# NyanCAD/CedarSim.jl

Hardware: AMD Instinct MI355X
Metric: newton_iters_per_sec (higher is better)
Workload: dtype f64

## Files before the change

### cedarsim.jl_amd/csrc/ch_persist.hpp

```cpp
#pragma once
#include <hip/hip_runtime.h>

#include "ch_kernels.hpp"

#ifdef CH_STAMPS
#define P_STAMP(slot) do { const unsigned long long now_ = __builtin_readcyclecounter(); pacc_[slot] += now_ - plast_; plast_ = now_; } while (0)
#else
#define P_STAMP(slot) do { } while (0)
#endif

namespace chip {

constexpr int PW = 4;
constexpr int P_MAXSRC = 64;
constexpr int P_NREC = 8;
constexpr int P_SCR = 64;
enum { PX_RUNNING = 0, PX_DONE = 1, PX_ROWS_FULL = 2, PX_ABORT = 3 };

struct TranCtl {
  double t, h;
  double tslot[8];
  int k, nhist, steps_at_order, reset_rate;
  int ibp, isave, status, exit_reason;
  long long nsaved, step;
// ... 29 lines not shown

struct PConst {
  const int* ci; const double* cd;
  __device__ int n_need() const { return ci[0]; }
  __device__ int n_ent() const { return ci[1]; }
  __device__ int n_pwl() const { return ci[2]; }
  __device__ const int* src_rec(int i) const { return ci + 4 + 3 * i; }
  __device__ const int* ent_ptr() const { return ci + 4 + 3 * n_need(); }
  __device__ const int* ent_idx() const { return ent_ptr() + n_ent() + 1; }
  __device__ const double* par(int i) const { return cd + 8 * i; }
  __device__ const double* ent_coef() const { return cd + 8 * n_need(); }
  __device__ const double* pwl_t() const { return ent_coef() + ent_ptr()[n_ent()]; }
  __device__ const double* pwl_y() const { return pwl_t() + n_pwl(); }
};

__device__ inline double p_pwl(const double* ts, const double* ys, int n, double t) {
  if (n == 0) return 0.0;
  int lo = 0, hi = n;
  while (lo < hi) { const int mid = (lo + hi) >> 1; if (ts[mid] < t) lo = mid + 1; else hi = mid; }
  int i = lo + 1;
  if (i <= n && ts[i - 1] == t) ++i;
  if (i <= 1) return ys[0];
  if (i > n) return ys[n - 1];
  const double y0 = ys[i - 2], y1 = ys[i - 1], t0 = ts[i - 2], t1 = ts[i - 1];
  if (y0 == y1) return y1;
  if (t1 == t0) return 0.5 * (y0 + y1);
  return y0 + (t - t0) * ((y1 - y0) / (t1 - t0));
}
__device__ inline double p_pwl4(double c0, double c1, double c2, double c3, double v1, double v2, double t) {
  int lb = (c0 < t) + (c1 < t) + (c2 < t) + (c3 < t);
  int i = lb + 1;
  const double tlb = lb == 0 ? c0 : lb == 1 ? c1 : lb == 2 ? c2 : c3;
  if (i <= 4 && tlb == t) ++i;
  if (i <= 1) return v1;
  if (i > 4) return v1;
  const double t0 = i == 2 ? c0 : i == 3 ? c1 : c2, t1 = i == 2 ? c1 : i == 3 ? c2 : c3;
  const double y0 = i == 2 ? v1 : v2, y1 = i == 4 ? v1 : v2;
  if (y0 == y1) return y1;
  if (t1 == t0) return 0.5 * (y0 + y1);
  return y0 + (t - t0) * ((y1 - y0) / (t1 - t0));
}
__device__ inline double p_source(const PConst& C, int i, double t) {
  const int* r = C.src_rec(i);
  const double* par = C.par(i);
  switch (r[0]) {
    case CH_SRC_DC: return par[0];
    case CH_SRC_PWL: return p_pwl(C.pwl_t() + r[1], C.pwl_y() + r[1], r[2], t);
    case CH_SRC_PULSE: {
      const double td = par[2], tr = par[3], tf = par[4], pw = par[5], per = par[6];
      const double tt = (per == per && fabs(per) < __builtin_inf()) ? fmod(t, per) : t;
      return p_pwl4(td, td + tr, td + tr + pw, td + tr + pw + tf, par[0], par[1], tt);
    }
    case CH_SRC_SIN: {
      const double vo = par[0], va = par[1], f = par[2], td = par[3], th = par[4], ph = par[5], nc = par[6];
      const double rad = 3.14159265358979323846 / 180.0;
      if (td < t && t < nc / f) return vo + va * exp(-(t - td) * th) * sin(fmod(360.0 * f * (t - td) + ph, 360.0) * rad);
      return vo + va * sin(fmod(ph, 360.0) * rad);
    }
  }
  return 0.0;
}

__device__ inline void p_source_piece(const PConst& C, int i, double t, double& t_lo, double& t_hi, double& y_lo, double& slope) {
  const int* r = C.src_rec(i);
  const double inf = __builtin_inf();
  t_lo = inf; t_hi = -inf; y_lo = 0.0; slope = 0.0;
  if (r[0] == CH_SRC_DC) { t_lo = -inf; t_hi = inf; y_lo = C.par(i)[0]; return; }
  if (r[0] != CH_SRC_PWL) return;
  const double* ts = C.pwl_t() + r[1]; const double* ys = C.pwl_y() + r[1];
  const int n = r[2];
  if (n == 0) { t_lo = -inf; t_hi = inf; return; }
  int lo = 0, hi = n;
  while (lo < hi) { const int mid = (lo + hi) >> 1; if (ts[mid] < t) lo = mid + 1; else hi = mid; }
  int k = lo + 1;
  if (k <= n && ts[k - 1] == t) ++k;
  if (k <= 1) { t_lo = -inf; t_hi = ts[0]; y_lo = ys[0]; return; }
  if (k > n) { t_lo = ts[n - 1]; t_hi = inf; y_lo = ys[n - 1]; return; }
  const double y0 = ys[k - 2], y1 = ys[k - 1], t0 = ts[k - 2], t1 = ts[k - 1];
  if (t1 == t0) return;
  t_lo = t0; t_hi = t1;
  if (y0 == y1) { y_lo = y1; slope = 0.0; } else { y_lo = y0; slope = (y1 - y0) / (t1 - t0); }
}

__device__ __forceinline__ void lds_fence() { asm volatile("s_waitcnt lgkmcnt(0)" ::: "memory"); }

__device__ __forceinline__ double ld_agent(const double* p) { return __hip_atomic_load(p, __ATOMIC_RELAXED, __HIP_MEMORY_SCOPE_AGENT); }
__device__ __forceinline__ void st_agent(double* p, double v) { __hip_atomic_store(p, v, __ATOMIC_RELAXED, __HIP_MEMORY_SCOPE_AGENT); }
__device__ __forceinline__ unsigned ld_agent_u(const unsigned* p) { return __hip_atomic_load(p, __ATOMIC_RELAXED, __HIP_MEMORY_SCOPE_AGENT); }

__device__ inline bool p_wait(const unsigned* cnt, unsigned target, unsigned* abort_flag, long long spin_ticks) {
  const long long t0 = wall_clock64();
  for (;;) {
    if (ld_agent_u(cnt) >= target) return true;
    if (ld_agent_u(abort_flag) != 0u) return false;
    if (wall_clock64() - t0 > spin_ticks) { __hip_atomic_store(abort_flag, 1u, __ATOMIC_RELAXED, __HIP_MEMORY_SCOPE_AGENT); return false; }
    __builtin_amdgcn_s_sleep(2);
  }
}

__device__ __forceinline__ double p_tree(double v, bool is_max) {
#pragma unroll
  for (int o = 8; o < 64; o <<= 1) { const double u = __shfl_xor(v, o); v = is_max ? fmax(v, u) : v + u; }
  return v;
}

typedef unsigned long long p_u64;
__device__ __forceinline__ p_u64 ld_gran(const p_u64* p) { return __hip_atomic_load(p, __ATOMIC_RELAXED, __HIP_MEMORY_SCOPE_AGENT); }
__device__ __forceinline__ void st_gran(p_u64* p, p_u64 v) { __hip_atomic_store(p, v, __ATOMIC_RELAXED, __HIP_MEMORY_SCOPE_AGENT); }
__device__ __forceinline__ double p_join(p_u64 gran, int lane) {
  const unsigned mine = (unsigned)gran, other = (unsigned)dpp_i<DPP_QP_1032>((int)mine);
  const unsigned lo = (lane & 1) ? other : mine, hi = (lane & 1) ? mine : other;
  return __hiloint2double((int)hi, (int)lo);
}
__device__ __forceinline__ p_u64 p_split(double v, int lane, unsigned gen) {
  const unsigned half = (lane & 1) ? (unsigned)__double2hiint(v) : (unsigned)__double2loint(v);
  return ((p_u64)gen << 32) | half;
}
__device__ __forceinline__ double p_rows4(double v, bool is_max, double* scr, int lane) {
  scr[lane] = v;
  asm volatile("s_waitcnt lgkmcnt(0)" ::: "memory");
  const int c = lane & 15;
  const double a0 = scr[c], a1 = scr[16 + c], a2 = scr[32 + c], a3 = scr[48 + c];
  asm volatile("s_waitcnt lgkmcnt(0)" ::: "memory");
  return is_max ? fmax(fmax(a0, a1), fmax(a2, a3)) : (a0 + a1) + (a2 + a3);
}
template <bool ALL_SUM = false>
__device__ inline bool p_grid_reduce(const PersistArgs& p, unsigned gen, const double* rec , double* part, double* summ,
                                     int* s_abort, int wave, int lane, int wg) {
  const int g16 = lane & 15, f = g16 >> 1, m4 = lane >> 4;
  const bool fmaxop = !ALL_SUM && ((f == 4) || (p.red_max && f < 3));
  if (lane < P_NREC) {
    double v = rec[0];
#pragma unroll
    for (int q = 1; q < P_NREC; ++q) v = (lane == q) ? rec[q] : v;
    part[wave * P_NREC + lane] = v;
  }
  __syncthreads();
  const int n_grp = p.n_wg < 8 ? p.n_wg : 8;
  const int grp = wg & 7;
  unsigned* abort_flag = p.counters + 9 * 32;
  p_u64* wrec = (p_u64*)p.wg_rec + (size_t)(gen & 1) * p.n_wg * 16;
  p_u64* grec = (p_u64*)p.grp_rec + (size_t)(gen & 1) * 8 * 16;
  double* scr = part + PW * P_NREC + P_NREC + 4;
  if (wave == 0) {
    bool ok = true;
    double v = part[f];
#pragma unroll
    for (int w = 1; w < PW; ++w) { const double u = part[w * P_NREC + f]; v = fmaxop ? fmax(v, u) : v + u; }
    if (p.n_wg > 1) {
      if (lane < 16) st_gran(wrec + (size_t)wg * 16 + g16, p_split(v, lane, gen));
      const long long t0 = wall_clock64();
      if (wg < n_grp) {
        const int members = (p.n_wg - grp + 7) >> 3;
        p_u64 x[8];
        for (;;) {
          bool all = true;
          const unsigned ab = ld_agent_u(abort_flag);
#pragma unroll
          for (int q = 0; q < 8; ++q) {
            const int mm = q * 4 + m4;
            x[q] = mm < members ? ld_gran(wrec + (size_t)(grp + 8 * mm) * 16 + g16) : ((p_u64)gen << 32);
            all = all && (unsigned)(x[q] >> 32) == gen;
          }
          if (__all(all)) break;
          if (ab != 0u) { ok = false; break; }
          if (wall_clock64() - t0 > p.spin_ticks) { __hip_atomic_store(abort_flag, 1u | (gen << 8), __ATOMIC_RELAXED, __HIP_MEMORY_SCOPE_AGENT); ok = false; break; }
          __builtin_amdgcn_s_sleep(1);
        }
        double acc = (m4 < members) ? p_join(x[0], lane) : 0.0;
#pragma unroll
        for (int q = 1; q < 8; ++q) {
          const double u = (q * 4 + m4 < members) ? p_join(x[q], lane) : 0.0;
          acc = fmaxop ? fmax(acc, u) : acc + u;
        }
        acc = p_rows4(acc, fmaxop, scr, lane);
        if (lane < 16) st_gran(grec + (size_t)grp * 16 + g16, p_split(acc, lane, gen));
      }
      p_u64 y[2];
      for (;;) {
        bool all = true;
        const unsigned ab = ok ? ld_agent_u(abort_flag) : 1u;
#pragma unroll
        for (int q = 0; q < 2; ++q) {
          const int gg = q * 4 + m4;
          y[q] = (ok && gg < n_grp) ? ld_gran(grec + (size_t)gg * 16 + g16) : ((p_u64)gen << 32);
          all = all && (unsigned)(y[q] >> 32) == gen;
        }
        if (__all(all) || !ok) break;
        if (ab != 0u) { ok = false; break; }
        if (wall_clock64() - t0 > p.spin_ticks) { __hip_atomic_store(abort_flag, 2u | (gen << 8), __ATOMIC_RELAXED, __HIP_MEMORY_SCOPE_AGENT); ok = false; break; }
        __builtin_amdgcn_s_sleep(1);
      }
      double acc = (m4 < n_grp) ? p_join(y[0], lane) : 0.0;
      { const double u = (4 + m4 < n_grp) ? p_join(y[1], lane) : 0.0; acc = fmaxop ? fmax(acc, u) : acc + u; }
      v = p_rows4(acc, fmaxop, scr, lane);
    }
    if (lane < 16 && !(lane & 1)) summ[f] = v;
    if (lane == 0) *s_abort = ok ? 0 : 1;
  }
  __syncthreads();
  return *s_abort == 0;
}

__device__ __forceinline__ double p_coef(double tau0, const double* tsl, int head, int kk, int np, int nkm1, int nkp1, bool lte, double hh, int lane, double& a0) {
  double tau[9];
  tau[0] = tau0;
#pragma unroll
  for (int i = 1; i < 9; ++i) tau[i] = tsl[(head - (i - 1)) & 7];
  const int set = lane >> 3, j = lane & 7;
  const double tj = j == 0 ? tau0 : tsl[(head - (j - 1)) & 7];
  const int n = set == 0 ? kk : set == 1 ? np : set == 2 ? nkm1 : set == 3 ? nkp1 : 0;
  const int lo = set == 0 ? 0 : 1;
  double num = 1.0, den = 1.0;
#pragma unroll
  for (int i = 0; i < 8; ++i) {
    const bool in_n = i >= 1 && i <= n && i != j, in_d = i >= lo && i <= n && i != j;
    num *= in_n ? tau[0] - tau[i] : 1.0;
    den *= in_d ? tj - tau[i] : 1.0;
  }
  if (!(set <= 3 && j >= 1 && j <= n)) { num = 0.0; den = 1.0; }
  double tk0 = tau[1], tk1 = tau[1], tk2 = tau[1];
#pragma unroll
  for (int i = 1; i < 9; ++i) { tk0 = (kk == i) ? tau[i] : tk0; tk1 = (kk + 1 == i) ? tau[i] : tk1; tk2 = (kk + 2 == i) ? tau[i] : tk2; }
  if (set == 4) {
    if (j >= 1 && j <= 5) { num = j <= kk ? 1.0 : 0.0; den = tau[0] - tj; }
    else if (j == 6) { num = lte ? hh : 0.0; den = tau[0] - tk1; }
    else if (j == 7) { num = nkm1 > 0 ? hh : 0.0; den = tau[0] - tk0; }
  } else if (set == 5 && j == 0) { num = nkp1 > 0 ? hh : 0.0; den = tau[0] - tk2; }
  if (num == 0.0) den = 1.0;
  const double q = num / den;
  a0 = bcast(row_sum<16>((set == 4 && j >= 1 && j <= 5) ? q : 0.0), 32);
  return q;
}

enum { PM_LOCKSTEP = 0, PM_OWN = 1, PM_BORDER = 2 };
template <int NC, bool PAIR, int MODE = PM_LOCKSTEP, bool WIDE = false>
__global__ __launch_bounds__(PW * 64, 1) void tran_persistent_kernel(const PersistArgs p) {
  typedef StampLayout<WIDE> SL;
  extern __shared__ double lds[];
  __shared__ int s_abort;
  __shared__ double s_bdec[4];
  const NewtonArgs& a = p.a;
  const int tid = threadIdx.x, lane = tid & 63, wave = tid >> 6, wg = blockIdx.x;
  const long long cyc0 = wall_clock64();
  long long cyc_bar = 0;
#ifdef CH_STAMPS
  unsigned long long pacc_[12] = {0, 0, 0, 0, 0, 0, 0, 0, 0, 0, 0, 0}, plast_ = __builtin_readcyclecounter();
#endif
  double* cdl = lds;
  int* cil = (int*)(cdl + p.n_cd);
  double* part = cdl + p.n_cd + ((p.n_ci + 1) >> 1);
  double* summ = part + PW * P_NREC;
  int* pfl = (int*)(summ + P_NREC);
  double* W = summ + P_NREC + 4 + P_SCR + (size_t)wave * p.wave_doubles;
  constexpr bool own = MODE == PM_OWN;
  const int* const wgc = own ? p.wgc : nullptr;
  const double* bps_own = nullptr; int nbp_own = 0;
  if (own && wgc) {
    const int* e = wgc + 6 * wg;
    const int* gci = p.ci + e[0]; const double* gcd = p.cd + e[1]; const int n_ci = e[2], n_cd = e[3];
    bps_own = p.bps + e[4]; nbp_own = e[5];
    for (int i = tid; i < n_cd; i += PW * 64) cdl[i] = gcd[i];
    for (int i = tid; i < n_ci; i += PW * 64) cil[i] = gci[i];
  } else {
    for (int i = tid; i < p.n_cd; i += PW * 64) cdl[i] = p.cd[i];
    for (int i = tid; i < p.n_ci; i += PW * 64) cil[i] = p.ci[i];
  }
#define P_BPS ((own && wgc) ? bps_own : p.bps)
#define P_NBP ((own && wgc) ? nbp_own : p.nbp)
  if (tid == 0) s_abort = 0;
  if (tid < 8) pfl[tid] = 0;
  __syncthreads();
  const PConst C{cil, cdl};

  const int blk = wg * p.bpw + wave;
  const bool live = wave < p.bpw && blk < p.nblk;
  const int bq = live ? blk : 0;
  const int c = bq / a.S, s = bq - c * a.S;
  const BlockMeta bm = a.bmeta[c];
  const ClassMeta cm = bm.cm;
  const int nc = cm.nc, ndev = cm.ndev, uofs = bm.uofs, dofs = bm.dofs, lda = nc + 1;
  double* st = W;
  double* A = st + (size_t)ndev * SL::STRIDE;
  double* Cm = A + (size_t)nc * lda;
  double* xl = Cm + (size_t)nc * nc;
  double* xp = xl + nc; double* Fv = xp + nc; double* Qv = Fv + nc; double* hq = Qv + nc;
  double* wv = hq + nc; double* qn = wv + nc; double* pm = qn + nc; double* pp = pm + nc; double* x0l = pp + nc;
  int* dml = (int*)(x0l + nc);
  double* Xh = x0l + 2 * nc; double* Qh = Xh + 8 * nc;
  double* tsl = Qh + 8 * nc; double* coef = tsl + 8;
  long long* stl = (long long*)(coef + 40);
  double* kvl = coef + 48; double* svl = kvl + (wgc ? C.ci[3] : a.nk);
  double* pl = wgc ? kvl + P_MAXSRC : svl + a.nsrc;
  int* mptr = (int*)(pl + (size_t)a.max_mc * B4L_STRIDE);
  int* slots = mptr + (nc * nc + 1) + (nc + 1);
  uint16_t* msrc = (uint16_t*)(slots + cm.nslots);
  const int2* wl = (const int2*)(mptr + cm.wl_ofs);
  const long sofs = (long)s * a.n_unk + uofs;
  const bool mine = live && lane < nc;
  const int role = wave & 1, pairq = wave >> 1, half = lane >> 5;
  int* pf = pfl + pairq * 4;
  const int blk_h = wg * p.bpw + (wave & ~1) + half;
  const bool live_h = PAIR && (wave & ~1) + half < p.bpw && blk_h < p.nblk;
  const int bqh = live_h ? blk_h : 0, c_h = bqh / a.S, s_h = bqh - c_h * a.S;
  const int uofs_h = PAIR ? a.bmeta[c_h].uofs : uofs, dofs_h = PAIR ? a.bmeta[c_h].dofs : dofs;
  double* Wh = summ + P_NREC + 4 + P_SCR + (size_t)((wave & ~1) + half) * p.wave_doubles;
  double* st_h = Wh; double* xl_h = Wh + (xl - W); double* pl_h = Wh + (pl - W);
  const int* slots_h = (const int*)((const char*)slots + ((const char*)Wh - (const char*)W));
  int pseq = 0; bool pair_broken = false;
  auto pair_sync = [&]() {
    ++pseq;
    lds_fence();
    if (lane == 0) __hip_atomic_store(pf + role, pseq, __ATOMIC_RELAXED, __HIP_MEMORY_SCOPE_WORKGROUP);
    const long long t0w = wall_clock64();
    while (__hip_atomic_load(pf + (1 - role), __ATOMIC_RELAXED, __HIP_MEMORY_SCOPE_WORKGROUP) < pseq) {
      if (wall_clock64() - t0w > p.spin_ticks) { pair_broken = true; __hip_atomic_store(p.counters + 9 * 32, 3u | ((unsigned)pseq << 8), __ATOMIC_RELAXED, __HIP_MEMORY_SCOPE_AGENT); break; }
      __builtin_amdgcn_s_sleep(0);
    }
    lds_fence();
  };

  if (live) {
    const int* bsrc = a.blob + cm.blob_ofs;
    for (int i = lane; i < cm.blob_ints; i += 64) mptr[i] = bsrc[i];
    const long scol = a.Smos > 1 ? s : 0;
    const int total = bm.mc_n * B4I_COUNT;
    for (int e = lane; e < total; e += 64) {
      const int j = e / B4I_COUNT, i = e - j * B4I_COUNT;
      int cl = bm.mc[0];
#pragma unroll
      for (int q = 1; q < 8; ++q) cl = (j == q) ? bm.mc[q] : cl;
      pl[j * B4L_STRIDE + i] = a.mosp[((long)cl * a.Smos + scol) * (long)B4I_COUNT + i];
    }
    for (int i = lane; i < nc * lda + nc * nc; i += 64) A[i] = 0.0;
    if (mine) {
      dml[lane] = a.dmask[uofs + lane] | ((a.unk_obs[uofs + lane] + 1) << 8);
#pragma unroll
      for (int j = 0; j < 7; ++j) {
        const bool have = j < p.ctl->nhist;
        Xh[((8 - j) & 7) * nc + lane] = have ? a.X[(long)j * a.slot_stride + sofs + lane] : 0.0;
        Qh[((8 - j) & 7) * nc + lane] = have ? a.Qh[(long)j * a.slot_stride + sofs + lane] : 0.0;
      }
      Xh[1 * nc + lane] = 0.0; Qh[1 * nc + lane] = 0.0;
    }
  }
  if (lane < 8) tsl[(8 - lane) & 7] = p.ctl->tslot[lane];
  double t, h; int k, nhist, steps_at_order, ibp, isave, status = CH_OK, exit_reason = PX_RUNNING;
  bool reset_rate;
  int nsaved, step;
  enum { ST_ACC = 0, ST_REJ, ST_FAIL, ST_ITERS, ST_BITERS, ST_ATT };
  int head = 0;
  {
    const TranCtl* cs = p.ctl;
    t = cs->t; h = cs->h; k = cs->k; nhist = cs->nhist; steps_at_order = cs->steps_at_order; reset_rate = cs->reset_rate != 0;
    ibp = cs->ibp; isave = cs->isave; nsaved = (int)cs->nsaved; step = (int)cs->step;
    if (lane == 0) { stl[ST_ACC] = cs->naccept; stl[ST_REJ] = cs->nreject; stl[ST_FAIL] = cs->nconvfail; stl[ST_ITERS] = cs->sum_iters; stl[ST_BITERS] = cs->sum_block_iters; stl[ST_ATT] = cs->n_attempts; }
  }
  double rate_prev = 1.0;
  int myrow = lane;
  if (MODE != PM_BORDER && a.perm && mine && p.resume) myrow = lane ^ (int)a.perm[(long)blk * 16 + lane];
  lds_fence();
  __syncthreads();

  const int s_e = PAIR ? s_h : s;
  const EvalCtx ectx{a.dkind, a.dterm, a.dsrc, a.dcls_local, a.dhdev, a.dpar, a.dmult, a.Spar, a.gmin_s[a.Sgmin > 1 ? s_e : 0],
                     WIDE ? a.vapar + (long)s_e * a.va_stride : a.vapar, WIDE ? a.temp_s[a.Stemp > 1 ? s_e : 0] + 273.15 : 300.15,
                     WIDE ? a.vacache + (long)s_e * a.vac_stride : nullptr, WIDE ? a.dvac : nullptr};
  const double gmin_h = a.gmin_s[a.Sgmin > 1 ? (PAIR ? s_h : s) : 0];
  SlotMeta smeta;
  int wslot = -1;
  if (WIDE) {
    smeta = load_slot_meta(ectx, 0, 0, 0, -1);
    if (PAIR) {
      const int sq = lane & 31;
      if (live_h) {
        if (sq < p.wide_l) wslot = slots_h[role == 0 ? sq : 64 + sq];
        else if (role == 0 && sq - p.wide_l < p.wide_other) wslot = slots_h[64 + p.wide_l + (sq - p.wide_l)];
      }
    } else if (live && lane < cm.nslots) wslot = slots[lane];
  }
  WideMeta wmeta = load_wide_meta(ectx, PAIR ? s_h : s, PAIR ? dofs_h : dofs, WIDE ? wslot : -1);
  bool va_lds = false;
  if (WIDE && p.va_arena > 0) {
    __shared__ unsigned long long s_va_ptr[32];
    __shared__ int s_va_ofs[32];
    __shared__ int s_va_n, s_va_top, s_va_fail;
    double* arena = summ + P_NREC + 4 + P_SCR + (size_t)PW * p.wave_doubles;
    if (tid == 0) { s_va_n = 0; s_va_top = 0; s_va_fail = 0; }
    __syncthreads();
    const double* staged[2] = {nullptr, nullptr};
    for (int w = 0; w < PW; ++w) {
      if (wave == w) {
#pragma unroll
        for (int which = 0; which < 2; ++which) {
          const double* g = which ? wmeta.C : wmeta.P;
          const int n = wmeta.mod < 0 ? 0 : (which ? va_gen::cache_doubles(wmeta.mod) : va_gen::param_doubles(wmeta.mod));
          bool pend = n > 0;
          for (;;) {
            const unsigned long long bal = __ballot(pend);
            if (!bal) break;
            const int srcl = __ffsll((long long)bal) - 1;
            const unsigned long long gp = ((unsigned long long)(unsigned)__shfl((int)((unsigned long long)g >> 32), srcl) << 32) | (unsigned)__shfl((int)(unsigned long long)g, srcl);
            const int nn = __shfl(n, srcl);
            const int ndir = s_va_n, top = s_va_top;
            int ofs = -1;
            for (int e = 0; e < ndir; ++e) if (s_va_ptr[e] == gp) ofs = s_va_ofs[e];
            if (ofs < 0 && ndir < 32 && top + nn <= p.va_arena) {
              ofs = top;
              const double* gsrc = (const double*)gp;
              for (int i = lane; i < nn; i += 64) arena[top + i] = gsrc[i];
              lds_fence();
              if (lane == 0) { s_va_ptr[ndir] = gp; s_va_ofs[ndir] = top; s_va_n = ndir + 1; s_va_top = top + ((nn + 1) & ~1); }
              lds_fence();
            }
            if (ofs < 0 && lane == 0) s_va_fail = 1;
            if (pend && (unsigned long long)g == gp) { staged[which] = ofs >= 0 ? arena + ofs : nullptr; pend = false; }
          }
        }
      }
      __syncthreads();
    }
    va_lds = s_va_fail == 0;
    if (va_lds && wmeta.mod >= 0) { wmeta.P = staged[0] ? staged[0] : arena; wmeta.C = staged[1] ? staged[1] : arena; }
  }
  if (!WIDE)
  {
    int slot = -1;
    if (PAIR) { const int sq = lane & 31; if (live_h && sq < cm.nslots) slot = slots_h[sq]; }
    else if (live && lane < cm.nslots) slot = slots[lane];
    smeta = load_slot_meta(ectx, PAIR ? s_h : s, PAIR ? dofs_h : dofs, PAIR ? uofs_h : uofs, slot);
    if (wgc && smeta.kind != 0) {
      const int* wk = p.wgk + (size_t)wg * P_MAXSRC;
      const int nkl = C.ci[3], nel = C.n_ent();
#pragma unroll
      for (int k = 0; k < 4; ++k) if (smeta.t[k] < 0) {
        const int g = -smeta.t[k] - 1; int j = 0;
        while (j < nkl - 1 && wk[j] != g) ++j;
        smeta.t[k] = -(j + 1);
      }
      if (smeta.kind == K_I || smeta.kind == K_V) { int j = nkl; while (j < nel - 1 && wk[j] != smeta.src) ++j; smeta.src = j - nkl; }
    }
  }
  const int n_ent = C.n_ent();
  const int e_p0 = lane < n_ent ? C.ent_ptr()[lane] : 0, e_nt = lane < n_ent ? C.ent_ptr()[lane + 1] - e_p0 : 0;
  const int e_i0 = e_nt > 0 ? C.ent_idx()[e_p0] : 0, e_i1 = e_nt > 1 ? C.ent_idx()[e_p0 + 1] : 0;
  const double e_c0 = e_nt > 0 ? C.ent_coef()[e_p0] : 0.0, e_c1 = e_nt > 1 ? C.ent_coef()[e_p0 + 1] : 0.0;
  double s0_lo = __builtin_inf(), s0_hi = -__builtin_inf(), s0_y = 0.0, s0_m = 0.0, s1_lo = __builtin_inf(), s1_hi = -__builtin_inf(), s1_y = 0.0, s1_m = 0.0;
  double bp_next = 0.0; int bp_at = -1;
  double bp_code = -1.0;
  double sv_next = 0.0; int sv_at = -1;
  const long long row_stride = (long long)p.n_obs * a.S;
  const int my_ob = mine ? (dml[lane] >> 8) - 1 : -1;
  unsigned gen = 0;

  if (!p.resume) {
    if (p.n_saveat == 0) {
      if (my_ob >= 0) p.out_rows[(long long)nsaved * row_stride + (long long)my_ob * a.S + s] = Xh[lane];
      if (blk == 0 && lane == 0) p.out_times[nsaved] = t;
      ++nsaved;
    } else {
      while (isave < p.n_saveat && p.saveat[isave] <= t) {
        if (my_ob >= 0) p.out_rows[(long long)nsaved * row_stride + (long long)my_ob * a.S + s] = Xh[lane];
        if (blk == 0 && lane == 0) p.out_times[nsaved] = p.saveat[isave];
        ++nsaved; ++isave;
      }
    }
  }

  P_STAMP(0);
  while (step < p.max_steps && t < p.t1) {
    if (p.n_saveat == 0 && nsaved >= p.max_rows) { exit_reason = PX_ROWS_FULL; break; }
    int ln = lane;
    asm volatile("" : "+v"(ln));
    for (;;) {
      if (bp_at != ibp) { bp_next = ibp < P_NBP ? P_BPS[ibp] : p.t1; bp_code = ibp < P_NBP ? P_BPS[P_NBP + ibp] : -1.0; bp_at = ibp; }
      if (ibp < P_NBP && bp_next <= t * (1 + 1e-15) + 1e-300) ++ibp; else break;
    }
    const double tb = bp_next;
    bool hit_bp = false;
    double tn = t + h;
    if (tn >= tb - 1e-3 * h) { tn = tb; hit_bp = true; }
    const double hh = tn - t;
    const bool dcm = MODE == PM_BORDER && p.dc_mode != 0;
    if (!dcm && hh < p.dtmin) { status = CH_ERR_DTMIN; break; }
    const int nh = nhist, kk = k < nh ? k : nh, np = (kk + 1) < nh ? (kk + 1) : nh;
    const bool lte = np >= kk + 1;
    const bool try_up = lte && kk < p.kmax && nh >= kk + 2 && steps_at_order + 1 >= kk + 1;
    const int nkm1 = (lte && kk > 1) ? kk : 0, nkp1 = try_up ? kk + 2 : 0;
    double alpha0;
    const double cq = p_coef(tn, tsl, head, kk, np, nkm1, nkp1, lte, hh, ln, alpha0);
    const double ck = bcast(cq, 38), ckm1 = bcast(cq, 39), ckp1 = bcast(cq, 40);
    if (dcm) alpha0 = 0.0;
    if (ln < 32) coef[ln] = cq;
    lds_fence();
    P_STAMP(1);
    {
      const double ts = (hit_bp && tn > 0.0) ? __longlong_as_double(__double_as_longlong(tn) - 1) : (hit_bp ? nextafter(tn, -__builtin_inf()) : tn);
      if (dcm) { if (lane < n_ent) kvl[lane] = p.dc_entries[lane]; }
      else if (lane < n_ent) {
        double v = 0.0;
        if (e_nt <= 2) {
          if (e_nt > 0) {
            if (!(s0_lo <= ts && ts < s0_hi)) p_source_piece(C, e_i0, ts, s0_lo, s0_hi, s0_y, s0_m);
            const double u = (s0_lo <= ts && ts < s0_hi) ? ((s0_m == 0.0) ? s0_y : s0_y + (ts - s0_lo) * s0_m) : p_source(C, e_i0, ts);
            v += e_c0 * u;
          }
          if (e_nt > 1) {
            if (!(s1_lo <= ts && ts < s1_hi)) p_source_piece(C, e_i1, ts, s1_lo, s1_hi, s1_y, s1_m);
            const double u = (s1_lo <= ts && ts < s1_hi) ? ((s1_m == 0.0) ? s1_y : s1_y + (ts - s1_lo) * s1_m) : p_source(C, e_i1, ts);
            v += e_c1 * u;
          }
        } else for (int q = e_p0; q < e_p0 + e_nt; ++q) v += C.ent_coef()[q] * p_source(C, C.ent_idx()[q], ts);
        kvl[lane] = v;
      }
    }
    P_STAMP(2);
    const int cand = (head + 1) & 7;
    double x0 = 0.0;
    {
      double pr = 0.0, hs = 0.0, m1 = 0.0, p1 = 0.0;
#pragma unroll
      for (int j = 0; j < 7; ++j) {
        const int sl = (head - j) & 7;
        const double xv = (mine && j < nh) ? Xh[sl * nc + lane] : 0.0;
        if (j == 0) x0 = xv;
        pr = fma(coef[8 + j + 1], xv, pr);
        m1 = fma(coef[16 + j + 1], xv, m1);
        p1 = fma(coef[24 + j + 1], xv, p1);
        if (j < 5) hs = fma(coef[j + 1], (mine && j < kk) ? Qh[sl * nc + lane] : 0.0, hs);
      }
      if (mine) {
        xp[lane] = pr; xl[lane] = pr; hq[lane] = hs; qn[lane] = 0.0; pm[lane] = m1; pp[lane] = p1;
        wv[lane] = 1.0 / (a.reltol * fabs(x0) + a.abstol);
      }
    }
    if (dcm && mine) { xp[lane] = x0; xl[lane] = x0; hq[lane] = 0.0; pm[lane] = x0; pp[lane] = x0; }
    lds_fence();
    P_STAMP(3);

    int nstat = 1, iters = 0;
    double rate_new = -1.0, dn_prev = 0.0;
    const double rp = reset_rate ? 1.0 : rate_prev;
    bool done_own = !live;
    constexpr bool bbd = MODE == PM_BORDER;
    const int no = nc - p.nb;
    bool stop_all = false, abort_all = false;
    bool dc_bad = false;
    double bA = 0.0, bB = 0.0, bC = 0.0, bN = 0.0;
    if (live || PAIR || bbd) {
      for (int it = 0; PAIR || bbd || it <= a.maxit; ++it) {
        if (bbd && stop_all) break;
        if (PAIR) {
          if (lane == 0) pf[2 + role] = done_own ? 1 : 0;
          pair_sync();
          const int d0 = pf[2], d1 = pf[3];
          if (!bbd && ((d0 && d1) || pair_broken)) break;
          if (!(half ? d1 : d0)) {
            if (WIDE) {
              if (wmeta.mod >= 0) { if (va_lds) eval_wide_cached<true>(wmeta, ectx, wslot, xl_h, uofs_h, kvl, st_h); else eval_wide_cached<false>(wmeta, ectx, wslot, xl_h, uofs_h, kvl, st_h); }
              else if (wslot >= 0) eval_slot<true>(ectx, s_h, dofs_h, wslot, xl_h, uofs_h, kvl, svl, pl_h, st_h);
            }
            else {
            if (role == 0) eval_cached<0>(smeta, gmin_h, xl_h, kvl, svl, pl_h, st_h);
            if (role == 1 ? (p.pair_dbg & 1) == 0 : (p.pair_dbg & 1) == 1) eval_cached<1>(smeta, gmin_h, xl_h, kvl, svl, pl_h, st_h);
            }
          }
          pair_sync();
          P_STAMP(4);
          if (!bbd) {
            if (pair_broken) break;
            if (done_own) continue;
          }
        } else {
        if (WIDE) {
          if (wmeta.mod >= 0) { if (va_lds) eval_wide_cached<true>(wmeta, ectx, wslot, xl, uofs, kvl, st); else eval_wide_cached<false>(wmeta, ectx, wslot, xl, uofs, kvl, st); }
          else if (wslot >= 0) eval_slot<true>(ectx, s, dofs, wslot, xl, uofs, kvl, svl, pl, st);
        }
        else if (!bbd || live) eval_cached<-1>(smeta, gmin_h, xl, kvl, svl, pl, st);
        lds_fence();
        P_STAMP(4);
        }
        for (int w = lane; w < ((bbd && !live) ? 0 : cm.n_work); w += 64) {
          const int2 itw = wl[w];
          const int p0 = itw.x, pe = p0 + (int)((unsigned)itw.y >> 16), e = itw.y & 0x7fff;
          const bool vec = itw.y & 0x8000;
          const int off2 = vec ? SL::QO : SL::CO;
          double s1 = 0.0, s2 = 0.0;
          for (int q = p0; q < pe; q += 4) {
            const int l = pe - 1;
            const int o0 = msrc[q], o1 = msrc[min(q + 1, l)], o2 = msrc[min(q + 2, l)], o3 = msrc[min(q + 3, l)];
            const double a0 = st[o0], b0 = st[o0 + off2], a1 = st[o1], b1 = st[o1 + off2], a2 = st[o2], b2 = st[o2 + off2], a3 = st[o3], b3 = st[o3 + off2];
            s1 += a0; s2 += b0;
            if (q + 1 < pe) { s1 += a1; s2 += b1; }
            if (q + 2 < pe) { s1 += a2; s2 += b2; }
            if (q + 3 < pe) { s1 += a3; s2 += b3; }
          }
          if (vec) {
            Qv[e] = s2;
            const double F = s1 + alpha0 * s2 + hq[e];
            Fv[e] = F;
            A[e * lda + nc] = -F;
          } else {
            const int r = e / nc, col = e - r * nc;
            A[r * lda + col] = s1 + alpha0 * s2;
            Cm[e] = s2;
          }
        }
        lds_fence();
        P_STAMP(5);
        constexpr int NCR = NC;
        double r[NCR + 1], cr[NCR];
        if constexpr (MODE == PM_BORDER) {
// ... 99 lines not shown
            const double dx = lu_bbd_back<NCR>(r, no, nc, lane, piv, mystep, ipiv, dxb0, dxb1);
            const double xn = xi + dx;
            if (mine) xl[lane] = xn;
            const bool bad = mine && (!(xn == xn) || fabs(xn) > 1e300);
            double q = Qi;
#pragma unroll
            for (int j = 0; j < NCR; ++j) if (j < nc) q = fma(cr[j], bcast(dx, j), q);
            if (mine) qn[lane] = q;
            const bool counted = mine && !(dml[lane] & 4);
            const double tq = dx * wi;
            e2own = bcast(row_sum<NCR>(counted ? tq * tq : 0.0), 0);
            lbad = __ballot(bad) ? 1.0 : 0.0;
            double v2k = 0.0, v2m = 0.0, v2p = 0.0, vnd = 0.0;
            if (counted && (dml[lane] & 1)) {
              const double w = 1.0 / (a.reltol * fmax(fabs(x0), fabs(xn)) + a.abstol);
              vnd = 1.0;
              double tq2 = (xn - xp[lane]) * w; v2k = tq2 * tq2;
              if (nkm1 > 0) { tq2 = (xn - pm[lane]) * w; v2m = tq2 * tq2; }
              if (nkp1 > 0) { tq2 = (xn - pp[lane]) * w; v2p = tq2 * tq2; }
            }
            l2k = bcast(row_sum<16>(v2k), 0); l2m = bcast(row_sum<16>(v2m), 0); l2p = bcast(row_sum<16>(v2p), 0); lnd = bcast(row_sum<16>(vnd), 0);
          }
          ++iters;
          double brec[P_NREC] = {l2k, l2m, l2p, lnd, e2own, lbad, 0.0, pair_broken ? 1.0 : 0.0};
          ++gen;
          const long long cbB = wall_clock64();
          okr = p_grid_reduce<true>(p, gen, brec, part, summ, &s_abort, wave, lane, wg);
          bA = summ[0]; bB = summ[1]; bC = summ[2]; bN = summ[3];
          const double e2g = summ[4]; const bool gbad = summ[5] != 0.0;
          if (!okr || summ[7] != 0.0) abort_all = true;
          __syncthreads();
          cyc_bar += wall_clock64() - cbB;
          if (abort_all) break;
          if (gbad) { nstat = 2; break; }
          const double dn = sqrt(e2g / (double)p.n_glob);
          if (it == 0) { if (dn <= a.newton_tol || (rp < 0.9 && 2.0 * fmax(rp, 0.02) * dn <= a.newton_tol)) { nstat = 0; stop_all = true; } }
          else { rate_new = dn_prev > 0.0 ? dn / dn_prev : 0.0; if (dn <= a.newton_tol) { nstat = 0; stop_all = true; } }
          dn_prev = dn;
          if (it + 1 >= a.maxit) stop_all = true;
          lds_fence();
          continue;
        }
        bool stop = false;
        if (!(fnorm == fnorm) || fnorm > 1e300) { nstat = 2; stop = true; }
        else if (it == a.maxit) { stop = true; }
        else {
          double dx = 0.0;
          P_STAMP(6);
          const bool ok = lu_solve_block<NCR>(A, lda, nc, lane, myrow, dx);
          P_STAMP(7);
          if (!ok) { nstat = 2; stop = true; }
          else {
            const double xn = xi + dx;
            if (mine) xl[lane] = xn;
            const bool bad = mine && (!(xn == xn) || fabs(xn) > 1e300);
            const double tq = dx * wi;
            const double e2 = bcast(row_sum<NCR>(mine ? tq * tq : 0.0), 0);
            const double q = RowDot<NCR, 0>::run(cr, dx, nc, Qi);
            if (mine) qn[lane] = q;
            ++iters;
            if (__ballot(bad)) { nstat = 2; stop = true; }
            else {
              const double dn = sqrt(e2 / nc);
              if (it == 0) { if (dn <= a.newton_tol || (rp < 0.9 && 2.0 * fmax(rp, 0.02) * dn <= a.newton_tol)) { nstat = 0; stop = true; } }
              else { rate_new = dn_prev > 0.0 ? dn / dn_prev : 0.0; if (dn <= a.newton_tol) { nstat = 0; stop = true; } }
              dn_prev = dn;
            }
          }
        }
        lds_fence();
        P_STAMP(8);
        if (stop) { if (PAIR) done_own = true; else break; }
      }
    }
    if (dcm) {
      if (abort_all) { exit_reason = PX_ABORT; status = CH_ERR_DEVICE; break; }
      if (mine) Xh[head * nc + lane] = xl[lane];
      if (lane == 0) { stl[ST_ITERS] += iters; stl[ST_BITERS] += (long long)iters * p.nblk; }
      lds_fence();
      status = nstat == 0 ? CH_OK : (nstat == 2 ? CH_ERR_SINGULAR : CH_ERR_MAXITERS);
      exit_reason = PX_DONE;
      break;
    }
    double e2k = 0.0, e2m = 0.0, e2p = 0.0, ndf = 0.0;
    if (mine) {
      const double xn = xl[lane];
      Xh[cand * nc + lane] = xn;
      Qh[cand * nc + lane] = qn[lane];
      if (dml[lane] & 1) {
        const double w = 1.0 / (a.reltol * fmax(fabs(x0), fabs(xn)) + a.abstol);
        ndf = 1.0;
        double tq = (xn - xp[lane]) * w; e2k = tq * tq;
        if (nkm1 > 0) { tq = (xn - pm[lane]) * w; e2m = tq * tq; }
        if (nkp1 > 0) { tq = (xn - pp[lane]) * w; e2p = tq * tq; }
      }
    }
    e2k = bcast(row_sum<16>(e2k), 0); e2m = bcast(row_sum<16>(e2m), 0); e2p = bcast(row_sum<16>(e2p), 0); ndf = bcast(row_sum<16>(ndf), 0);
    if ((live || bbd) && nstat == 0) rate_prev = iters >= 2 ? fmin(1.0, fmax(rate_new, 1e-4)) : fmin(1.0, rp * 1.5);
    double rec[P_NREC];
    if (p.red_max) { const double inv = ndf > 0.0 ? 1.0 / ndf : 0.0; rec[0] = e2k * inv; rec[1] = e2m * inv; rec[2] = e2p * inv; }
    else { rec[0] = e2k; rec[1] = e2m; rec[2] = e2p; }
    rec[3] = ndf; rec[4] = (double)iters; rec[5] = (double)iters; rec[6] = (live && nstat != 0) ? 1.0 : 0.0; rec[7] = 0.0;
    if (!live) { for (int q = 0; q < P_NREC; ++q) rec[q] = 0.0; }
    if (pair_broken) rec[7] = 1.0;
    if (!bbd) ++gen;
    P_STAMP(9);
    const long long cb0 = wall_clock64();
    double sA, sB, sC, sN, sItMax, sItSum, sFail;
    if (own) {
      double r8[P_NREC];
#pragma unroll
      for (int q = 0; q < P_NREC; ++q) r8[q] = rec[q];
      if (PAIR) {
        if (lane < P_NREC) { double v = rec[0];
#pragma unroll
          for (int q = 1; q < P_NREC; ++q) v = (lane == q) ? rec[q] : v;
          part[wave * P_NREC + lane] = v; }
        pair_sync();
        const double* other = part + (wave ^ 1) * P_NREC;
#pragma unroll
        for (int q = 0; q < P_NREC; ++q) { const double o = other[q]; r8[q] = (q < 3 || q == 4) ? fmax(r8[q], o) : r8[q] + o; }
        if (pair_broken) r8[7] = 1.0;
      }
      sA = r8[0]; sB = r8[1]; sC = r8[2]; sN = r8[3]; sItMax = r8[4]; sItSum = (double)iters; sFail = r8[6];
      if (r8[7] != 0.0) { exit_reason = PX_ABORT; status = CH_ERR_DEVICE; break; }
    } else if (bbd) {
      if (abort_all) { exit_reason = PX_ABORT; status = CH_ERR_DEVICE; break; }
      sA = bA; sB = bB; sC = bC; sN = bN; sItMax = (double)iters; sItSum = (double)iters * (double)p.nblk; sFail = nstat != 0 ? 1.0 : 0.0;
    } else {
      const bool okr = p_grid_reduce(p, gen, rec, part, summ, &s_abort, wave, lane, wg);
      if (!okr || summ[7] != 0.0) { exit_reason = PX_ABORT; status = CH_ERR_DEVICE; break; }
      sA = summ[0]; sB = summ[1]; sC = summ[2]; sN = summ[3]; sItMax = summ[4]; sItSum = summ[5]; sFail = summ[6];
      __syncthreads();
    }
    cyc_bar += wall_clock64() - cb0;
    P_STAMP(10);
    double errk, errkm1, errkp1;
    double ev3;
    {
      const double sv = ln == 0 ? sA : ln == 1 ? sB : sC, cv = ln == 0 ? ck : ln == 1 ? ckm1 : ckp1;
      ev3 = p.red_max ? cv * sqrt(sv) : (sN > 0.0 ? cv * sqrt(sv / sN) : 0.0);
      errk = bcast(ev3, 0); errkm1 = bcast(ev3, 1); errkp1 = bcast(ev3, 2);
    }
    if (lane == 0) { stl[ST_ATT] += 1; stl[ST_BITERS] += (long long)sItSum; stl[ST_ITERS] += p.red_max ? (long long)sItSum : (long long)sItMax; }
    if (sFail > 0.0) {
      if (lane == 0) stl[ST_FAIL] += 1;
      reset_rate = true;
      h = hh * 0.25; k = 1; steps_at_order = 0;
      if (nhist > 2) nhist = 2;
      P_STAMP(11);
      continue;
    }
    if (!lte) errk = 0.0;
    double fk, fm, fp;
    {
      const double ev = (ln == 0 && !lte) ? 0.0 : ev3;
      const double ex = ln == 0 ? (double)(kk + 1) : ln == 1 ? (double)kk : (double)(kk + 2);
      const double fv = exp(-flog(2.0 * ev + 1e-4) / ex);
      fk = bcast(fv, 0); fm = bcast(fv, 1); fp = bcast(fv, 2);
    }
    if (errk > 1.0) {
      if (lane == 0) stl[ST_REJ] += 1;
      h = hh * fmin(0.9, fmax(0.25, 0.9 * fk));
      steps_at_order = 0;
      P_STAMP(11);
      continue;
    }
    if (lane == 0) stl[ST_ACC] += 1;
    ++step; reset_rate = false;
    head = cand;
    if (lane == 0) tsl[head] = tn;
    lds_fence();
    nhist = nhist + 1 < p.kmax + 2 ? nhist + 1 : p.kmax + 2;
    if (p.n_saveat > 0) {
      for (;;) {
        if (sv_at != isave) { sv_next = isave < p.n_saveat ? p.saveat[isave] : __builtin_inf(); sv_at = isave; }
        if (!(isave < p.n_saveat && sv_next <= tn * (1 + 1e-15))) break;
        const double tsv = sv_next;
        const int msv = (kk < nh ? kk : nh) + 1;
        double dummy;
        const double wq = p_coef(tsv, tsl, head, 0, msv, 0, 0, false, 0.0, ln, dummy);
        if (ln < 32) coef[ln] = wq;
        lds_fence();
        double v = 0.0;
#pragma unroll
        for (int j = 0; j < 7; ++j) v = fma(coef[8 + j + 1], (mine && j < msv) ? Xh[((head - j) & 7) * nc + lane] : 0.0, v);
        lds_fence();
        if (my_ob >= 0) p.out_rows[(long long)nsaved * row_stride + (long long)my_ob * a.S + s] = v;
        if (blk == 0 && lane == 0) p.out_times[nsaved] = tsv;
        ++nsaved; ++isave;
      }
    } else {
      if (my_ob >= 0) p.out_rows[(long long)nsaved * row_stride + (long long)my_ob * a.S + s] = Xh[head * nc + lane];
      if (blk == 0 && lane == 0) { p.out_times[nsaved] = tn; p.out_times[p.max_rows + nsaved] = (double)((kk < nh ? kk : nh) + 1); }
      ++nsaved;
    }
    double best = fk; int knew = kk;
    if (lte) {
      ++steps_at_order;
      if (kk > 1 && fm > best) { best = fm; knew = kk - 1; }
      if (try_up && fp > 1.1 * best) { best = fp; knew = kk + 1; }
    } else knew = 1;
    if (knew != kk) steps_at_order = 0;
    k = knew;
    if (best > 1.0 && best < 1.2) best = 1.0;
    h = fmin(p.dtmax, hh * fmin(kk == 1 ? 10.0 : 2.0, fmax(0.5, best)));
    t = tn;
    if (hit_bp && t < p.t1) {
      reset_rate = true;
      if (bp_code < 0) {
        nhist = 1; k = 1; steps_at_order = 0;
        double nb = p.t1;
        for (int b = ibp; b < P_NBP; ++b) if (P_BPS[b] > t * (1 + 1e-15)) { nb = P_BPS[b]; break; }
        h = fmax(p.dtmin * 10, fmin(h, (nb - t) / 50.0) * p.first_frac);
      } else h = fmax(p.dtmin * 10, fmin(h, bp_code * 0.1));
    }
    P_STAMP(11);
  }
  if (exit_reason == PX_RUNNING) {
    exit_reason = PX_DONE;
    if (status == CH_OK && t < p.t1) status = CH_ERR_MAXSTEPS;
  }
  if (MODE != PM_BORDER && a.perm && mine) a.perm[(long)blk * 16 + lane] = (unsigned char)(myrow ^ lane);
  if (mine) {
#pragma unroll
    for (int j = 0; j < 7; ++j) {
      const int sl = (head - j) & 7;
      a.X[(long)j * a.slot_stride + sofs + lane] = Xh[sl * nc + lane];
      a.Qh[(long)j * a.slot_stride + sofs + lane] = Qh[sl * nc + lane];
    }
  }
  if (own) {
    if (live && lane == 0) {
      TranCtl* cs = p.ctl + 1;
      typedef unsigned long long u64;
      atomicAdd((u64*)&cs->sum_iters, (u64)stl[ST_ITERS]); atomicAdd((u64*)&cs->sum_block_iters, (u64)stl[ST_BITERS]);
      atomicMax((u64*)&cs->naccept, (u64)stl[ST_ACC]); atomicMax((u64*)&cs->nreject, (u64)stl[ST_REJ]); atomicMax((u64*)&cs->nconvfail, (u64)stl[ST_FAIL]);
      atomicMax((u64*)&cs->n_attempts, (u64)stl[ST_ATT]); atomicMax((u64*)&cs->nsaved, (u64)nsaved); atomicMax((u64*)&cs->max_iters, (u64)stl[ST_ITERS]);
      atomicMin(&cs->status, status); atomicMax(&cs->exit_reason, exit_reason);
      if (blk == 0) { cs->t = t; cs->h = h; cs->isave = isave; cs->t_cycles_total = wall_clock64() - cyc0; cs->t_cycles_barrier = cyc_bar; }
    }
  } else
  if (wg == 0 && wave == 0 && lane == 0) {
    TranCtl* cs = p.ctl;
    cs->t = t; cs->h = h; cs->k = k; cs->nhist = nhist; cs->steps_at_order = steps_at_order; cs->reset_rate = reset_rate ? 1 : 0;
    cs->ibp = ibp; cs->isave = isave; cs->status = status; cs->exit_reason = exit_reason; cs->nsaved = nsaved; cs->step = step;
    cs->naccept = stl[ST_ACC]; cs->nreject = stl[ST_REJ]; cs->nconvfail = stl[ST_FAIL]; cs->sum_iters = stl[ST_ITERS]; cs->sum_block_iters = stl[ST_BITERS]; cs->n_attempts = stl[ST_ATT];
    for (int j = 0; j < 8; ++j) cs->tslot[j] = tsl[(head - j) & 7];
    cs->t_cycles_total = wall_clock64() - cyc0; cs->t_cycles_barrier = cyc_bar;
#ifdef CH_STAMPS
    for (int q = 0; q < 12; ++q) cs->stamps[q] = (long long)pacc_[q];
#endif
  }
}

#undef P_BPS
#undef P_NBP

}
```

Baseline: 50480.

## Slim persistent kernel hot paths: outline cold source lookups, bitmask coefficients, cheaper spin

Moves PWL source miss handling and the dense saveat coefficient path into noinline cold functions to shrink the hot loop's code and register footprint. Rewrites p_coef with bitmask-driven products and lane-range selection instead of nested per-lane conditionals. Caches the error-norm count and the ck/ckm1/ckp1 coefficients in LDS instead of recomputing with reductions and broadcasts, and hoists history row pointers using a scalar nc. The pair spin-wait now reads the wall clock only every 64 trips, and the unused p_wait helper is removed. Together these trade some extra LDS traffic and call overhead on rare paths for less per-step VALU and register pressure.

```diff
diff --git a/cedarsim.jl_amd/csrc/ch_persist.hpp b/cedarsim.jl_amd/csrc/ch_persist.hpp
--- a/cedarsim.jl_amd/csrc/ch_persist.hpp
+++ b/cedarsim.jl_amd/csrc/ch_persist.hpp
@@ -135,21 +135,22 @@
   if (y0 == y1) { y_lo = y1; slope = 0.0; } else { y_lo = y0; slope = (y1 - y0) / (t1 - t0); }
 }
 
+__device__ __attribute__((noinline, cold)) double p_source_cold(const int* ci, const double* cd, int i, double t) { return p_source(PConst{ci, cd}, i, t); }
+struct PPiece { double lo, hi, y, m, u; };
+__device__ __attribute__((noinline, cold)) PPiece p_source_miss(const int* ci, const double* cd, int i, double ts) {
+  PPiece q;
+  p_source_piece(PConst{ci, cd}, i, ts, q.lo, q.hi, q.y, q.m);
+  q.u = (q.lo <= ts && ts < q.hi) ? ((q.m == 0.0) ? q.y : q.y + (ts - q.lo) * q.m) : p_source_cold(ci, cd, i, ts);
+  return q;
+}
+
 __device__ __forceinline__ void lds_fence() { asm volatile("s_waitcnt lgkmcnt(0)" ::: "memory"); }
 
 __device__ __forceinline__ double ld_agent(const double* p) { return __hip_atomic_load(p, __ATOMIC_RELAXED, __HIP_MEMORY_SCOPE_AGENT); }
 __device__ __forceinline__ void st_agent(double* p, double v) { __hip_atomic_store(p, v, __ATOMIC_RELAXED, __HIP_MEMORY_SCOPE_AGENT); }
 __device__ __forceinline__ unsigned ld_agent_u(const unsigned* p) { return __hip_atomic_load(p, __ATOMIC_RELAXED, __HIP_MEMORY_SCOPE_AGENT); }
 
-__device__ inline bool p_wait(const unsigned* cnt, unsigned target, unsigned* abort_flag, long long spin_ticks) {
-  const long long t0 = wall_clock64();
-  for (;;) {
-    if (ld_agent_u(cnt) >= target) return true;
-    if (ld_agent_u(abort_flag) != 0u) return false;
-    if (wall_clock64() - t0 > spin_ticks) { __hip_atomic_store(abort_flag, 1u, __ATOMIC_RELAXED, __HIP_MEMORY_SCOPE_AGENT); return false; }
-    __builtin_amdgcn_s_sleep(2);
-  }
-}
+constexpr unsigned P_SPIN_CLOCK = 64;
 
 __device__ __forceinline__ double p_tree(double v, bool is_max) {
 #pragma unroll
@@ -256,34 +257,37 @@
 }
 
 __device__ __forceinline__ double p_coef(double tau0, const double* tsl, int head, int kk, int np, int nkm1, int nkp1, bool lte, double hh, int lane, double& a0) {
-  double tau[9];
+  double tau[8];
   tau[0] = tau0;
 #pragma unroll
-  for (int i = 1; i < 9; ++i) tau[i] = tsl[(head - (i - 1)) & 7];
+  for (int i = 1; i < 8; ++i) tau[i] = tsl[(head - (i - 1)) & 7];
   const int set = lane >> 3, j = lane & 7;
-  const double tj = j == 0 ? tau0 : tsl[(head - (j - 1)) & 7];
-  const int n = set == 0 ? kk : set == 1 ? np : set == 2 ? nkm1 : set == 3 ? nkp1 : 0;
-  const int lo = set == 0 ? 0 : 1;
+  const int npk = kk | (np << 4) | (nkm1 << 8) | (nkp1 << 12);
+  const int n = set <= 3 ? (npk >> (4 * set)) & 15 : 0;
+  const bool act = set <= 3 && j >= 1 && j <= n;
+  const unsigned mn = act ? ((2u << n) - 2u) & ~(1u << j) : 0u;
+  const unsigned md = mn | ((act && set == 0) ? 1u : 0u);
+  const bool rcp = lane >= 33 && lane <= 37, cks = lane >= 38 && lane <= 40;
+  const int pick = lane == 38 ? kk + 1 : lane == 39 ? kk : kk + 2;
+  const int m = cks ? ((pick >= 1 && pick <= 8) ? pick : 1) : j;
+  const double tj = tsl[(head - (m - 1)) & 7];
   double num = 1.0, den = 1.0;
 #pragma unroll
   for (int i = 0; i < 8; ++i) {
-    const bool in_n = i >= 1 && i <= n && i != j, in_d = i >= lo && i <= n && i != j;
-    num *= in_n ? tau[0] - tau[i] : 1.0;
-    den *= in_d ? tj - tau[i] : 1.0;
-  }
-  if (!(set <= 3 && j >= 1 && j <= n)) { num = 0.0; den = 1.0; }
-  double tk0 = tau[1], tk1 = tau[1], tk2 = tau[1];
-#pragma unroll
-  for (int i = 1; i < 9; ++i) { tk0 = (kk == i) ? tau[i] : tk0; tk1 = (kk + 1 == i) ? tau[i] : tk1; tk2 = (kk + 2 == i) ? tau[i] : tk2; }
-  if (set == 4) {
-    if (j >= 1 && j <= 5) { num = j <= kk ? 1.0 : 0.0; den = tau[0] - tj; }
-    else if (j == 6) { num = lte ? hh : 0.0; den = tau[0] - tk1; }
-    else if (j == 7) { num = nkm1 > 0 ? hh : 0.0; den = tau[0] - tk0; }
-  } else if (set == 5 && j == 0) { num = nkp1 > 0 ? hh : 0.0; den = tau[0] - tk2; }
+    num *= ((mn >> i) & 1u) ? tau[0] - tau[i] : 1.0;
+    den *= ((md >> i) & 1u) ? tj - tau[i] : 1.0;
+  }
+  if (!act) { num = 0.0; den = 1.0; }
+  const bool on = rcp ? j <= kk : lane == 38 ? lte : lane == 39 ? nkm1 > 0 : nkp1 > 0;
+  if (rcp || cks) { num = on ? (rcp ? 1.0 : hh) : 0.0; den = tau[0] - tj; }
   if (num == 0.0) den = 1.0;
   const double q = num / den;
-  a0 = bcast(row_sum<16>((set == 4 && j >= 1 && j <= 5) ? q : 0.0), 32);
+  a0 = bcast(row_sum<16>(rcp ? q : 0.0), 32);
   return q;
+}
+__device__ __attribute__((noinline, cold)) double p_coef_dense(double tsv, const double* tsl, int head, int msv, int lane) {
+  double a0;
+  return p_coef(tsv, tsl, head, 0, msv, 0, 0, false, 0.0, lane, a0);
 }
 
 enum { PM_LOCKSTEP = 0, PM_OWN = 1, PM_BORDER = 2 };
@@ -351,6 +355,7 @@
   const int2* wl = (const int2*)(mptr + cm.wl_ofs);
   const long sofs = (long)s * a.n_unk + uofs;
   const bool mine = live && lane < nc;
+  const int nc_s = __builtin_amdgcn_readfirstlane(nc);
   const int role = wave & 1, pairq = wave >> 1, half = lane >> 5;
   int* pf = pfl + pairq * 4;
   const int blk_h = wg * p.bpw + (wave & ~1) + half;
@@ -365,9 +370,13 @@
     ++pseq;
     lds_fence();
     if (lane == 0) __hip_atomic_store(pf + role, pseq, __ATOMIC_RELAXED, __HIP_MEMORY_SCOPE_WORKGROUP);
-    const long long t0w = wall_clock64();
-    while (__hip_atomic_load(pf + (1 - role), __ATOMIC_RELAXED, __HIP_MEMORY_SCOPE_WORKGROUP) < pseq) {
-      if (wall_clock64() - t0w > p.spin_ticks) { pair_broken = true; __hip_atomic_store(p.counters + 9 * 32, 3u | ((unsigned)pseq << 8), __ATOMIC_RELAXED, __HIP_MEMORY_SCOPE_AGENT); break; }
+    long long t0w = 0;
+    for (unsigned trip = 1; __hip_atomic_load(pf + (1 - role), __ATOMIC_RELAXED, __HIP_MEMORY_SCOPE_WORKGROUP) < pseq; ++trip) {
+      if (trip % P_SPIN_CLOCK == 0u) {
+        const long long now = wall_clock64();
+        if (trip == P_SPIN_CLOCK) t0w = now;
+        else if (now - t0w > p.spin_ticks) { pair_broken = true; __hip_atomic_store(p.counters + 9 * 32, 3u | ((unsigned)pseq << 8), __ATOMIC_RELAXED, __HIP_MEMORY_SCOPE_AGENT); break; }
+      }
       __builtin_amdgcn_s_sleep(0);
     }
     lds_fence();
@@ -398,6 +407,10 @@
     }
   }
   if (lane < 8) tsl[(8 - lane) & 7] = p.ctl->tslot[lane];
+  {
+    const double nd = row_sum<16>((mine && (dml[lane] & 1)) ? 1.0 : 0.0);
+    if (lane == 0) coef[35] = nd;
+  }
   double t, h; int k, nhist, steps_at_order, ibp, isave, status = CH_OK, exit_reason = PX_RUNNING;
   bool reset_rate;
   int nsaved, step;
@@ -542,9 +555,8 @@
     const int nkm1 = (lte && kk > 1) ? kk : 0, nkp1 = try_up ? kk + 2 : 0;
     double alpha0;
     const double cq = p_coef(tn, tsl, head, kk, np, nkm1, nkp1, lte, hh, ln, alpha0);
-    const double ck = bcast(cq, 38), ckm1 = bcast(cq, 39), ckp1 = bcast(cq, 40);
     if (dcm) alpha0 = 0.0;
-    if (ln < 32) coef[ln] = cq;
+    if (ln < 32 || (ln >= 38 && ln <= 40)) coef[ln < 32 ? ln : ln - 6] = cq;
     lds_fence();
     P_STAMP(1);
     {
@@ -554,16 +566,18 @@
         double v = 0.0;
         if (e_nt <= 2) {
           if (e_nt > 0) {
-            if (!(s0_lo <= ts && ts < s0_hi)) p_source_piece(C, e_i0, ts, s0_lo, s0_hi, s0_y, s0_m);
-            const double u = (s0_lo <= ts && ts < s0_hi) ? ((s0_m == 0.0) ? s0_y : s0_y + (ts - s0_lo) * s0_m) : p_source(C, e_i0, ts);
+            double u;
+            if (s0_lo <= ts && ts < s0_hi) u = (s0_m == 0.0) ? s0_y : s0_y + (ts - s0_lo) * s0_m;
+            else { const PPiece q = p_source_miss(C.ci, C.cd, e_i0, ts); s0_lo = q.lo; s0_hi = q.hi; s0_y = q.y; s0_m = q.m; u = q.u; }
             v += e_c0 * u;
           }
           if (e_nt > 1) {
-            if (!(s1_lo <= ts && ts < s1_hi)) p_source_piece(C, e_i1, ts, s1_lo, s1_hi, s1_y, s1_m);
-            const double u = (s1_lo <= ts && ts < s1_hi) ? ((s1_m == 0.0) ? s1_y : s1_y + (ts - s1_lo) * s1_m) : p_source(C, e_i1, ts);
+            double u;
+            if (s1_lo <= ts && ts < s1_hi) u = (s1_m == 0.0) ? s1_y : s1_y + (ts - s1_lo) * s1_m;
+            else { const PPiece q = p_source_miss(C.ci, C.cd, e_i1, ts); s1_lo = q.lo; s1_hi = q.hi; s1_y = q.y; s1_m = q.m; u = q.u; }
             v += e_c1 * u;
           }
-        } else for (int q = e_p0; q < e_p0 + e_nt; ++q) v += C.ent_coef()[q] * p_source(C, C.ent_idx()[q], ts);
+        } else for (int q = e_p0; q < e_p0 + e_nt; ++q) v += C.ent_coef()[q] * p_source_cold(C.ci, C.cd, C.ent_idx()[q], ts);
         kvl[lane] = v;
       }
     }
@@ -572,15 +586,18 @@
     double x0 = 0.0;
     {
       double pr = 0.0, hs = 0.0, m1 = 0.0, p1 = 0.0;
+      const double* xr = Xh + (mine ? lane : 0);
+      const double* qr = Qh + (mine ? lane : 0);
 #pragma unroll
       for (int j = 0; j < 7; ++j) {
-        const int sl = (head - j) & 7;
-        const double xv = (mine && j < nh) ? Xh[sl * nc + lane] : 0.0;
+        const int so = ((head - j) & 7) * nc_s;
+        const double xj = xr[so], qj = j < 5 ? qr[so] : 0.0;
+        const double xv = (mine && j < nh) ? xj : 0.0;
         if (j == 0) x0 = xv;
         pr = fma(coef[8 + j + 1], xv, pr);
         m1 = fma(coef[16 + j + 1], xv, m1);
         p1 = fma(coef[24 + j + 1], xv, p1);
-        if (j < 5) hs = fma(coef[j + 1], (mine && j < kk) ? Qh[sl * nc + lane] : 0.0, hs);
+        if (j < 5) hs = fma(coef[j + 1], (mine && j < kk) ? qj : 0.0, hs);
       }
       if (mine) {
         xp[lane] = pr; xl[lane] = pr; hq[lane] = hs; qn[lane] = 0.0; pm[lane] = m1; pp[lane] = p1;
@@ -846,20 +863,20 @@
       exit_reason = PX_DONE;
       break;
     }
-    double e2k = 0.0, e2m = 0.0, e2p = 0.0, ndf = 0.0;
+    double e2k = 0.0, e2m = 0.0, e2p = 0.0;
     if (mine) {
       const double xn = xl[lane];
       Xh[cand * nc + lane] = xn;
       Qh[cand * nc + lane] = qn[lane];
       if (dml[lane] & 1) {
         const double w = 1.0 / (a.reltol * fmax(fabs(x0), fabs(xn)) + a.abstol);
-        ndf = 1.0;
         double tq = (xn - xp[lane]) * w; e2k = tq * tq;
         if (nkm1 > 0) { tq = (xn - pm[lane]) * w; e2m = tq * tq; }
         if (nkp1 > 0) { tq = (xn - pp[lane]) * w; e2p = tq * tq; }
       }
     }
-    e2k = bcast(row_sum<16>(e2k), 0); e2m = bcast(row_sum<16>(e2m), 0); e2p = bcast(row_sum<16>(e2p), 0); ndf = bcast(row_sum<16>(ndf), 0);
+    e2k = bcast(row_sum<16>(e2k), 0); e2m = bcast(row_sum<16>(e2m), 0); e2p = bcast(row_sum<16>(e2p), 0);
+    const double ndf = coef[35];
     if ((live || bbd) && nstat == 0) rate_prev = iters >= 2 ? fmin(1.0, fmax(rate_new, 1e-4)) : fmin(1.0, rp * 1.5);
     double rec[P_NREC];
     if (p.red_max) { const double inv = ndf > 0.0 ? 1.0 / ndf : 0.0; rec[0] = e2k * inv; rec[1] = e2m * inv; rec[2] = e2p * inv; }
@@ -902,7 +919,7 @@
     double errk, errkm1, errkp1;
     double ev3;
     {
-      const double sv = ln == 0 ? sA : ln == 1 ? sB : sC, cv = ln == 0 ? ck : ln == 1 ? ckm1 : ckp1;
+      const double sv = ln == 0 ? sA : ln == 1 ? sB : sC, cv = coef[32 + (ln < 2 ? ln : 2)];
       ev3 = p.red_max ? cv * sqrt(sv) : (sN > 0.0 ? cv * sqrt(sv / sN) : 0.0);
       errk = bcast(ev3, 0); errkm1 = bcast(ev3, 1); errkp1 = bcast(ev3, 2);
     }
@@ -942,8 +959,7 @@
         if (!(isave < p.n_saveat && sv_next <= tn * (1 + 1e-15))) break;
         const double tsv = sv_next;
         const int msv = (kk < nh ? kk : nh) + 1;
-        double dummy;
-        const double wq = p_coef(tsv, tsl, head, 0, msv, 0, 0, false, 0.0, ln, dummy);
+        const double wq = p_coef_dense(tsv, tsl, head, msv, ln);
         if (ln < 32) coef[ln] = wq;
         lds_fence();
         double v = 0.0;
```

After: 52060 (median of 6 runs). +3.1%, better.
